# isl-org/Open3D

Measured on AMD Instinct MI355X. Metric: RGB-D frames/s, TSDF integrate with known poses (configs[1]: touch + activate + integrate into an 8 mm / 16^3 VoxelBlockGrid); the ICP + integrate + ray-cast loop (configs[2]) is in loop_frames_per_s (its first tracked frame untimed as warm-up; the whole run in loop_frames_per_s_with_first_frame), higher is better.
Workload: dtype f32; 1 GPU; block_count=50000, frames_per_launch=12, active_blocks=5745

## Files before the change

### open3d_amd/csrc/host/voxel_block_grid.cpp

```cpp

#include <cctype>
#include <chrono>
#include <cstdio>
#include <cstdlib>
#include <cstring>
#include <string>
#include <vector>

#include "../common.h"
#include "../npz.h"
#include "../stream_path.h"
#include "../sliced_path.h"
#include "../touch_device.h"
#include "../collectives.h"
#include "o3d_mi355x_host.h"

using namespace o3dmi;

struct o3dmi_vbg {
    float voxel_size = 0;
    int64_t block_resolution = 0;
    std::vector<std::string> attr_names;
    std::vector<int> attr_dtypes;
    std::vector<int> attr_channels;
// ... 1000 lines not shown
    int64_t seq = 0;
    int stamp = 0;
    const StreamFrame* frames = nullptr;
};

static StreamGroup MakeGroup(o3dmi_vbg* g, const StreamCommon& c,
                             const StreamFrame* frames, int n,
                             FrameFrontArgs* fa) {
    StreamGroup grp;
    grp.n = n;
    grp.seq = g->stream_seq;
    g->frame_stamp += 1;
    grp.stamp = g->frame_stamp;
    grp.frames = frames;
    const int par = (int)(grp.seq & 1);
    for (int f = 0; f < n; ++f) {
        FrameFrontArgs& a = fa[f];
        a.depth = (const uint16_t*)frames[f].depth;
        a.color = c.with_color ? (const uint8_t*)frames[f].color : nullptr;
        a.rows = c.depth_rows;
        a.cols = c.depth_cols;
        a.color_rows = c.color_rows;
        a.color_cols = c.color_cols;
        a.depth_intrinsic = c.depth_intrinsic;
        a.color_intrinsic = c.color_intrinsic ? c.color_intrinsic
                                              : c.depth_intrinsic;
        a.extrinsic = frames[f].extrinsic;
        a.resolution = (int)g->block_resolution;
        a.voxel_size = g->voxel_size;
        a.sdf_trunc = g->voxel_size * c.trunc;
        a.depth_scale = c.depth_scale;
        a.depth_max = c.depth_max;
        a.stride = 4;
        a.group_stamp = (unsigned long long)grp.stamp;
        a.group_bit = f;
        a.touch_plane = par;
        a.col_lut = g->prep_valid ? g->prep_col : nullptr;
        a.row_lut = g->prep_valid ? g->prep_row : nullptr;
        a.depth_div_short = g->prep_valid && g->prep_div_short;
        a.prep_identity = g->prep_valid && g->prep_identity;
        a.recs = g->recs[par][f];
        a.list = g->lists[par];
        a.list_capacity = g->lists_capacity;
        a.count = g->ring_counters + (grp.seq & 3);
        a.ready = g->ready[par];
        a.tickets = g->front_tickets + 16 * par;
        a.touch_status = (int*)g->stream_status + 4;
        a.prepare_only = false;
    }
    g->stream_seq += 1;
    g->size_bound = o3dmi_hash_capacity(g->block_hashmap);
    return grp;
}

static void MakeIntegArgs(o3dmi_vbg* g, const StreamCommon& c,
                          const StreamGroup& grp, bool prof,
                          IntegrateStreamArgs* ia) {
    const int par = (int)(grp.seq & 1);
    ia->n_frames = grp.n;
    ia->group_stamp = (unsigned long long)grp.stamp;
    ia->touch_plane = par;
    for (int f = 0; f < grp.n; ++f) {
        ia->recs[f] = g->recs[par][f];
        ia->extrinsic[f] = grp.frames[f].extrinsic;
    }
    ia->rows = c.depth_rows;
    ia->cols = c.depth_cols;
    ia->with_color = c.with_color;
    ia->list = g->lists[par];
    ia->ready = g->ready[par];
    ia->count = g->ring_counters + (grp.seq & 3);
    ia->list_capacity = g->lists_capacity;
    ia->grid_hint = g->last_count;
    ia->tsdf = (float*)o3dmi_hash_value_buffer(g->block_hashmap, c.ti);
    ia->weight = o3dmi_hash_value_buffer(g->block_hashmap, c.wi);
    ia->color = c.with_color ? o3dmi_hash_value_buffer(g->block_hashmap, c.ci)
                             : nullptr;
    ia->grid_dtype = c.grid_dtype;
    ia->depth_intrinsic = c.depth_intrinsic;
    ia->resolution = (int)g->block_resolution;
    ia->voxel_size = g->voxel_size;
    ia->sdf_trunc = g->voxel_size * c.trunc;
    ia->depth_max = c.depth_max;
    ia->zero_counter = g->ring_counters + ((grp.seq + 2) & 3);
    ia->size_host = (int*)g->stream_status;
    ia->status_stamp = grp.stamp;
    ia->prof_count = prof ? g->prof_counts + g->prof_max + g->prof_frames
                          : nullptr;
    ia->prof_frame_blocks = prof ? g->prof_counts + g->prof_frames : nullptr;
    ia->prof_map_size =
            prof ? g->prof_counts + 2 * g->prof_max + g->prof_frames : nullptr;
}

static bool StreamPathApplies(const o3dmi_vbg* g, int input_dtype) {
    int ti = g->AttrIndex("tsdf"), wi = g->AttrIndex("weight");
    return input_dtype == O3DMI_U16 && (g->block_resolution % 4) == 0 &&
           ti >= 0 && wi >= 0 && g->attr_dtypes[(size_t)ti] == O3DMI_F32;
}

static int WaitTouchReported(o3dmi_vbg* g, int stamp, hipStream_t s,
                             int* overflow) {
    const auto t0 = std::chrono::steady_clock::now();
    for (;;) {
        int st = PollStreamStatus(g, overflow);
        if (st) return st;
        if (*overflow != 0 || g->touch_seen_stamp - stamp >= 0) return O3DMI_OK;
        if (std::chrono::steady_clock::now() - t0 >
            std::chrono::milliseconds(20)) {
            O3DMI_HIP_CHECK(hipStreamSynchronize(s));
            if ((st = PollStreamStatus(g, overflow))) return st;
            return O3DMI_OK;
        }
    }
}

static int StreamIntegrate(o3dmi_vbg* g, const StreamCommon& c0,
                           const StreamFrame* frames, int n, int group,
                           hipStream_t s) {
    StreamCommon c = c0;
    if (group < 1) group = 1;
    if (group > kMaxGroup) group = kMaxGroup;
    c.frame_new = FrustumBlockBound(
            c.depth_intrinsic, c.depth_rows, c.depth_cols, c.depth_max,
            g->voxel_size * (float)g->block_resolution, 4);
    O3DMI_REQUIRE(c.frame_new > 0, "depth image too small");
    const int64_t group_new = c.frame_new * group;
    c.ti = g->AttrIndex("tsdf");
    c.wi = g->AttrIndex("weight");
    c.ci = g->AttrIndex("color");
    c.with_color = c.ci >= 0 && (int64_t)c.color_rows * c.color_cols > 0 &&
                   n > 0 && frames[0].color != nullptr;
    int st = GridDtype(g, &c.grid_dtype);
    if (st) return st;
    if ((st = EnsureStreamBuffers(g, c.depth_rows, c.depth_cols,
                                  c.frame_new * kMaxGroup)))
        return st;

    if ((st = EnsurePrepTables(g, c.depth_intrinsic, c.color_intrinsic,
                                      c.depth_rows, c.depth_cols,
                                      c.color_rows, c.color_cols,
                                      c.depth_scale, s))) {
        return st;
    }
    (void)PrefetchFastDivision(g->voxel_size * c.trunc, n == 1);
    static const bool strict_only =
            std::getenv("O3DMI_STRICT_CAPACITY") != nullptr;
    const bool allow_est = !strict_only && n > 1;

    struct Pending {
        int stamp, f0;
    };
    std::vector<Pending> pending;
    bool issued = false;
    StreamGroup cur;
    FrameFrontArgs fa[kMaxGroup];
    int f = 0;
    for (;;) {
        int overflow = 0;
        while (f < n && overflow == 0) {
            if (!issued) {
                Issue how;
                if ((st = StreamEnsureCapacity(g, group_new, allow_est, s,
                                               &how, &overflow)))
                    return st;
                if (overflow != 0) break;
                const int m = n - f < group ? n - f : group;
// ... 1876 lines not shown
```

### open3d_amd/csrc/stream_path.h

```cpp
#pragma once

#include "common.h"

namespace o3dmi {

constexpr int kMaxGroup = 16;
static_assert(kMaxGroup == kTouchBits, "one touch bit per frame of a group");
constexpr int kDefaultGroup = 8;
constexpr int kGroupChunk = 4;

struct alignas(16) FrameBlock {
    int slot, x, y, z;
};

struct alignas(16) ReadyEntry {
    unsigned long long key;
    int block_idx;
    unsigned bits;
};

struct alignas(8) PixelRec {
    float d;
    unsigned rgba;
};

struct FrameFrontArgs {
    const uint16_t* depth;
    const uint8_t* color;
    int rows, cols, color_rows, color_cols;
    const double* depth_intrinsic;
    const double* color_intrinsic;
    const double* extrinsic;
    int resolution;
    float voxel_size, sdf_trunc, depth_scale, depth_max;
    int stride;
    unsigned long long group_stamp;
    int group_bit;
    int touch_plane;
    const int* col_lut;
    const int* row_lut;
    bool depth_div_short;
    bool prep_identity;
    PixelRec* recs;
    FrameBlock* list;
    int64_t list_capacity;
    int* count;
    ReadyEntry* ready;
    int* tickets;
    int* touch_status;
    bool prepare_only;
};

struct IntegrateStreamArgs {
    int n_frames;
    unsigned long long group_stamp;
    int touch_plane;
    const PixelRec* recs[kMaxGroup];
    const double* extrinsic[kMaxGroup];
    int rows, cols;
    bool with_color;
    const FrameBlock* list;
    const ReadyEntry* ready;
    const int* count;
    int64_t list_capacity;
    int grid_hint;
    float* tsdf;
    void* weight;
    void* color;
    int grid_dtype;
    const double* depth_intrinsic;
    int resolution;
    float voxel_size, sdf_trunc, depth_max;
    int* zero_counter;
    int* size_host;
    int status_stamp;
    int* prof_count;
    int* prof_frame_blocks;
    int* prof_map_size;
};

int LaunchFrameStep(o3dmi_hash* block_hash, const FrameFrontArgs* fronts,
                    int n_fronts, const IntegrateStreamArgs* integ,
                    hipStream_t s);

int PrefetchFastDivision(float sdf_trunc, bool wait);

int RecoverOverflow(o3dmi_hash* block_hash, hipStream_t s, int64_t* wanted);

bool PrepTables(const double* depth_intrinsic, const double* color_intrinsic,
                int rows, int cols, int color_rows, int color_cols,
                float depth_scale, int* col, int* row);

int64_t FrustumBlockBound(const double* intrinsic, int rows, int cols,
                          float depth_max, float block_size, int stride);

}
```

### open3d_amd/csrc/vbg_stream.hip

```cpp

#include <cmath>

#include "common.h"
#include <cmath>
#include <cstdio>
#include <cstdlib>
#include <cstring>
#include <map>
#include <mutex>
#include <string>

#include "stream_path.h"
#include "sliced_path.h"
#include "touch_device.h"

#ifndef O3DMI_ABLATE_GATHER
#define O3DMI_ABLATE_GATHER 0
#endif

namespace o3dmi {
namespace {

template <typename T, int N, int A>
struct alignas(A) Vec {
    T v[N];
};

__device__ __forceinline__ float DivByConst(float a, float b, float y) {
    const float q0 = a * y;
    const float r = __builtin_fmaf(-b, q0, a);
    return __builtin_fmaf(r, y, q0);
}
struct PrepParams {
    Camera color_cam;
    int color_rows, color_cols;
    bool with_color;
};

constexpr int kTileKeys = 2048;

struct FrontShared {
    TouchParams p;
    PrepParams pp;
    const int* col_lut;
    const int* row_lut;
    bool depth_div_short;
    bool prep_identity;
    float inv_depth_scale;
    FrameBlock* list;
    int64_t list_capacity;
    int* out_count;
    ReadyEntry* ready;
    int* tickets;
    int* touch_status;
    int n_touch_total;
    unsigned long long group_stamp;
    int touch_plane;
    int n_touch_wg, n_prep_wg;
};
inline bool SameIntrinsics(const Camera& a, const Camera& b) {
    return a.fx == b.fx && a.fy == b.fy && a.cx == b.cx && a.cy == b.cy &&
           a.scale == b.scale;
}
inline bool SameGroup(const FrontShared& a, const FrontShared& b) {
    return SameIntrinsics(a.p.cam, b.p.cam) && a.p.rows == b.p.rows &&
           a.p.cols == b.p.cols && a.p.stride == b.p.stride &&
           a.p.rows_strided == b.p.rows_strided &&
           a.p.cols_strided == b.p.cols_strided &&
           a.p.block_size == b.p.block_size &&
           a.p.sdf_trunc == b.p.sdf_trunc &&
           a.p.depth_scale == b.p.depth_scale &&
           a.p.depth_max == b.p.depth_max &&
           SameIntrinsics(a.pp.color_cam, b.pp.color_cam) &&
           a.pp.color_rows == b.pp.color_rows &&
           a.pp.color_cols == b.pp.color_cols &&
           a.pp.with_color == b.pp.with_color && a.col_lut == b.col_lut &&
           a.row_lut == b.row_lut && a.depth_div_short == b.depth_div_short &&
           a.prep_identity == b.prep_identity &&
           a.inv_depth_scale == b.inv_depth_scale && a.list == b.list &&
           a.list_capacity == b.list_capacity && a.out_count == b.out_count &&
           a.ready == b.ready && a.tickets == b.tickets &&
           a.touch_status == b.touch_status &&
           a.n_touch_total == b.n_touch_total &&
           a.group_stamp == b.group_stamp && a.touch_plane == b.touch_plane &&
           a.n_touch_wg == b.n_touch_wg && a.n_prep_wg == b.n_prep_wg;
}
struct FrontFrame {
    float pose[3][4];
    const uint16_t* depth;
    const uint8_t* color;
    PixelRec* recs;
    int group_bit;
};

struct FrontParams {
    TouchParams p;
    PrepParams pp;
    const uint16_t* depth;
    const uint8_t* color;
    const int* col_lut;
    const int* row_lut;
    bool depth_div_short;
    bool prep_identity;
    float inv_depth_scale;
    PixelRec* recs;
    FrameBlock* list;
    int64_t list_capacity;
    int* out_count;
    ReadyEntry* ready;
    int* tickets;
    int* touch_status;
    int n_touch_total;
    unsigned long long group_stamp;
    int group_bit;
    int touch_plane;
// ... 104 lines not shown
                    __hip_atomic_store(fp.out_count, 0, __ATOMIC_RELAXED,
                                       __HIP_MEMORY_SCOPE_AGENT);
            }
            if (threadIdx.x == 0 && fp.touch_status) {
                const int top = __hip_atomic_load(&hv.counters[0],
                                                  __ATOMIC_RELAXED,
                                                  __HIP_MEMORY_SCOPE_AGENT);
                fp.touch_status[0] = top < hv.capacity ? top : hv.capacity;
                fp.touch_status[1] = overflow;
                fp.touch_status[2] = n;
                __hip_atomic_store(&fp.touch_status[3], (int)fp.group_stamp,
                                   __ATOMIC_RELEASE, __HIP_MEMORY_SCOPE_SYSTEM);
            }
            const auto make_entry = [&](int i) -> ReadyEntry {
                const unsigned long long* e =
                        reinterpret_cast<const unsigned long long*>(&list[i]);
                const unsigned long long lo = __hip_atomic_load(
                        e, __ATOMIC_RELAXED, __HIP_MEMORY_SCOPE_AGENT);
                const unsigned long long hi = __hip_atomic_load(
                        e + 1, __ATOMIC_RELAXED, __HIP_MEMORY_SCOPE_AGENT);
                const unsigned slot = (unsigned)lo;
                const int x = (int)(unsigned)(lo >> 32);
                const int y = (int)(unsigned)hi, z = (int)(unsigned)(hi >> 32);
                const int idx = __hip_atomic_load(&hv.slot_vals[slot],
                                                  __ATOMIC_RELAXED,
                                                  __HIP_MEMORY_SCOPE_AGENT);
                const unsigned long long word = __hip_atomic_load(
                        TouchWord(hv, slot, fp.touch_plane), __ATOMIC_RELAXED,
                        __HIP_MEMORY_SCOPE_AGENT);
                const bool own = (word >> kTouchBits) == fp.group_stamp;
                if (!own) atomicOr(&hv.counters[1], kErrTouchStamp);
                ReadyEntry re;
                re.key = PackKey(x, y, z);
                re.block_idx = idx;
                re.bits = own ? (unsigned)(word & ((1ull << kTouchBits) - 1ull))
                              : 0u;
                return re;
            };
            constexpr int kPerLane = 4;
            const int kSortable = kPerLane * (int)blockDim.x;
            __shared__ int s_bins[kTouchBits + 2];
            if (n <= kSortable) {
                if (threadIdx.x < kTouchBits + 2) s_bins[threadIdx.x] = 0;
                __syncthreads();
                ReadyEntry mine[kPerLane];
                int pc[kPerLane];
#pragma unroll
                for (int k = 0; k < kPerLane; ++k) {
                    const int i = (int)threadIdx.x + k * (int)blockDim.x;
                    pc[k] = -1;
                    if (i < n) {
                        mine[k] = make_entry(i);
                        pc[k] = __popc(mine[k].bits);
                    }
                }
#pragma unroll
                for (int k = 0; k < kPerLane; ++k)
                    if (pc[k] >= 0) atomicAdd(&s_bins[pc[k]], 1);
                __syncthreads();
                if (threadIdx.x == 0) {
                    int run = 0;
                    for (int b = kTouchBits; b >= 0; --b) {
                        const int c = s_bins[b];
                        s_bins[b] = run;
                        run += c;
                    }
                }
                __syncthreads();
#pragma unroll
                for (int k = 0; k < kPerLane; ++k)
                    if (pc[k] >= 0)
                        fp.ready[atomicAdd(&s_bins[pc[k]], 1)] = mine[k];
            } else {
                for (int i = threadIdx.x; i < n; i += blockDim.x)
                    fp.ready[i] = make_entry(i);
            }
        }
        return;
    }
    const int n_px = p.rows * p.cols;
    const int n_wg = fp.n_prep_wg;
    if (wg == n_touch_wg && threadIdx.x == 0) {
        PixelRec r;
        r.d = 0.0f;
        r.rgba = 0u;
        recs[n_px] = r;
    }
    if (fp.col_lut && fp.prep_identity) {
        const int n_groups = n_px >> 2;
        const int gstep = n_wg * blockDim.x;
        constexpr int kG = 4;
        for (int g0 = (wg - n_touch_wg) * blockDim.x + threadIdx.x;
             g0 < n_groups; g0 += kG * gstep) {
            uint2 dq[kG];
            unsigned cw[kG][3];
#pragma unroll
            for (int k = 0; k < kG; ++k) {
                const int g = g0 + k * gstep;
                const int gc = g < n_groups ? g : n_groups - 1;
                dq[k] = *reinterpret_cast<const uint2*>(depth + 4 * (int64_t)gc);
                if (pp.with_color) {
                    const unsigned* c = reinterpret_cast<const unsigned*>(
                            color + 12 * (int64_t)gc);
                    cw[k][0] = c[0];
                    cw[k][1] = c[1];
                    cw[k][2] = c[2];
                }
            }
#pragma unroll
            for (int k = 0; k < kG; ++k) {
                const int g = g0 + k * gstep;
                if (g >= n_groups) continue;
                const unsigned dv[4] = {dq[k].x & 0xffffu, dq[k].x >> 16,
                                        dq[k].y & 0xffffu, dq[k].y >> 16};
                unsigned rgba[4] = {0u, 0u, 0u, 0u};
                if (pp.with_color) {
                    rgba[0] = (cw[k][0] & 0xffffffu) | (1u << 24);
                    rgba[1] = ((cw[k][0] >> 24) | ((cw[k][1] & 0xffffu) << 8)) |
                              (1u << 24);
                    rgba[2] = ((cw[k][1] >> 16) | ((cw[k][2] & 0xffu) << 16)) |
                              (1u << 24);
                    rgba[3] = (cw[k][2] >> 8) | (1u << 24);
                }
                uint4 o[2];
                unsigned w[8];
#pragma unroll
                for (int j = 0; j < 4; ++j) {
                    const float df = (float)dv[j];
                    const float d =
                            fp.depth_div_short
                                    ? DivByConst(df, p.depth_scale,
                                                 fp.inv_depth_scale)
                                    : df / p.depth_scale;
                    w[2 * j] = __float_as_uint(d);
                    w[2 * j + 1] = rgba[j];
                }
                o[0] = make_uint4(w[0], w[1], w[2], w[3]);
                o[1] = make_uint4(w[4], w[5], w[6], w[7]);
                uint4* dst = reinterpret_cast<uint4*>(recs + 4 * (int64_t)g);
                dst[0] = o[0];
                dst[1] = o[1];
            }
        }
        return;
    }
    if (fp.col_lut) {
        const int* __restrict__ col_lut = fp.col_lut;
        const int* __restrict__ row_lut = fp.row_lut;
        const int step = n_wg * blockDim.x;
        const int step_v = step / p.cols, step_u = step - step_v * p.cols;
        for (int first = (wg - n_touch_wg) * blockDim.x + threadIdx.x;
             first < n_px; first += 4 * step) {
            int idx[4], uc[4], vc[4];
            float df[4];
#pragma unroll
            for (int k = 0; k < 4; ++k) {
                const int i = first + k * step;
                idx[k] = i < n_px ? i : n_px - 1;
                df[k] = (float)depth[idx[k]];
            }
            if (pp.with_color) {
                int vi = first / p.cols;
                int ui = first - vi * p.cols;
#pragma unroll
                for (int k = 0; k < 4; ++k) {
                    uc[k] = col_lut[ui];
                    vc[k] = row_lut[vi < p.rows ? vi : p.rows - 1];
                    ui += step_u;
                    vi += step_v;
                    if (ui >= p.cols) {
                        ui -= p.cols;
                        ++vi;
                    }
                }
            }
            unsigned rgba[4] = {0u, 0u, 0u, 0u};
            if (pp.with_color) {
                unsigned c0[4], c1[4], c2[4];
#pragma unroll
                for (int k = 0; k < 4; ++k) {
                    const bool has = (uc[k] | vc[k]) >= 0;
                    const uint8_t* in =
                            color + (has ? ((int64_t)vc[k] * pp.color_cols +
                                            uc[k]) * 3
                                         : 0);
                    c0[k] = in[0];
                    c1[k] = in[1];
                    c2[k] = in[2];
                }
#pragma unroll
                for (int k = 0; k < 4; ++k)
                    rgba[k] = (uc[k] | vc[k]) >= 0
                                      ? (c0[k] | (c1[k] << 8) | (c2[k] << 16) |
                                         (1u << 24))
                                      : 0u;
            }
#pragma unroll
            for (int k = 0; k < 4; ++k) {
                PixelRec r;
                r.d = fp.depth_div_short
                              ? DivByConst(df[k], p.depth_scale,
                                           fp.inv_depth_scale)
                              : df[k] / p.depth_scale;
                r.rgba = rgba[k];
                if (first + k * step < n_px) recs[idx[k]] = r;
            }
        }
        return;
    }
    for (int i = (wg - n_touch_wg) * blockDim.x + threadIdx.x; i < n_px;
         i += n_wg * blockDim.x) {
        const int vi = i / p.cols;
        const int ui = i - vi * p.cols;
        PixelRec r;
        r.d = (float)depth[i] / p.depth_scale;
        r.rgba = 0u;
        if (pp.with_color) {
            float x, y, z, uf, vf;
            p.cam.Unproject((float)ui, (float)vi, 1.0f, x, y, z);
            pp.color_cam.Project(x, y, z, uf, vf);
            if (InBoundary2D(uf, vf, pp.color_rows, pp.color_cols)) {
                int uc = (int)roundf(uf);
                int vc = (int)roundf(vf);
                const uint8_t* in =
                        color + ((int64_t)vc * pp.color_cols + uc) * 3;
                r.rgba = (unsigned)in[0] | ((unsigned)in[1] << 8) |
                         ((unsigned)in[2] << 16) | (1u << 24);
            }
        }
        recs[i] = r;
    }
}

struct IntegParams {
    Camera cam0;
    float ext[kMaxGroup][3][4];
    const PixelRec* recs[kMaxGroup];
    int n_frames;
    unsigned long long group_stamp;
    int touch_plane;
    int rows, cols, resolution;
    int res_shift;
    int cube;
    float sdf_trunc, depth_max;
    float inv_sdf_trunc;
    const FrameBlock* list;
    const ReadyEntry* ready;
    const int* count;
    int64_t list_capacity;
    float* tsdf;
    void* weight;
    void* color;
    int* zero_counter;
    int* size_host;
    int status_stamp;
    int* prof_count;
    unsigned long long* prof_items;
    int* prof_frame_blocks;
    int* prof_map_size;
    const uint16_t* raw_depth[kMaxGroup];
    const uint8_t* raw_color[kMaxGroup];
    float depth_scale, inv_depth_scale;
    bool depth_div_short;
    const ChunkEntry* entries;
    const IntegFrame* frame_tab;
};

__device__ __forceinline__ float RcpSmallInt(float b) {
    const float r0 = __builtin_amdgcn_rcpf(b);
    const float e = __builtin_fmaf(-b, r0, 1.0f);
    return __builtin_fmaf(e, r0, r0);
}

constexpr float kDivTiny = 1.0e-30f;

__device__ __forceinline__ float DivByConstGuarded(float a, float b, float y) {
    if (__builtin_amdgcn_ballot_w64(fabsf(a) < kDivTiny) != 0ull) return a / b;
    return DivByConst(a, b, y);
}

__global__ void VerifyDivKernel(float b, float y, unsigned max_bits,
                                int* __restrict__ mismatch) {
    int bad = 0;
    for (unsigned long long i = blockIdx.x * (unsigned long long)blockDim.x +
                                threadIdx.x;
         i <= max_bits; i += (unsigned long long)gridDim.x * blockDim.x) {
        const float a = __uint_as_float((unsigned)i);
        const float want_p = a / b, want_n = (-a) / b;
        const float got_p = DivByConstGuarded(a, b, y);
        const float got_n = DivByConstGuarded(-a, b, y);
        if (__float_as_uint(want_p) != __float_as_uint(got_p) ||
            __float_as_uint(want_n) != __float_as_uint(got_n))
            bad |= 1;
    }
    if (bad) atomicOr(mismatch, bad);
}
template <int kSteps>
__device__ __forceinline__ float RcpGuarded(float z) {
    const bool out = (__float_as_uint(z) - 0x21800000u) >= (0x5E000000u - 0x21800000u);
    if (__builtin_amdgcn_ballot_w64(out) != 0ull) return 1.0f / z;
    float r = __builtin_amdgcn_rcpf(z);
#pragma unroll
    for (int k = 0; k < kSteps; ++k) {
        const float e = __builtin_fmaf(-z, r, 1.0f);
        r = __builtin_fmaf(e, r, r);
    }
    return r;
}
__device__ __forceinline__ bool RcpOutOfRange(float z) {
    return (__float_as_uint(z) - 0x21800000u) >= (0x5E000000u - 0x21800000u);
}
template <int kSteps>
__device__ __forceinline__ float RcpNewton(float z) {
    float r = __builtin_amdgcn_rcpf(z);
#pragma unroll
    for (int k = 0; k < kSteps; ++k) {
        const float e = __builtin_fmaf(-z, r, 1.0f);
        r = __builtin_fmaf(e, r, r);
    }
    return r;
}
template <int kSteps>
__global__ void VerifyRcpZKernel(int* __restrict__ mismatch, int bit) {
    const unsigned lo = 0x21000000u, hi = 0x5E800000u;
    bool bad = false;
    for (unsigned long long i = lo + blockIdx.x * (unsigned long long)blockDim.x +
                                threadIdx.x;
         i <= hi; i += (unsigned long long)gridDim.x * blockDim.x) {
        const float z = __uint_as_float((unsigned)i);
        bad |= __float_as_uint(1.0f / z) !=
               __float_as_uint(RcpGuarded<kSteps>(z));
    }
    if (bad) atomicOr(mismatch, bit);
}

__global__ void VerifyRcpKernel(int* __restrict__ mismatch) {
    const int i = blockIdx.x * blockDim.x + threadIdx.x + 1;
    if (i > 65536) return;
    const float b = (float)i;
    if (__float_as_uint(1.0f / b) != __float_as_uint(RcpSmallInt(b)))
        atomicOr(mismatch, 2);
}

typedef float f2 __attribute__((ext_vector_type(2)));

__device__ __forceinline__ f2 Splat(float a) { return f2{a, a}; }
__device__ __forceinline__ f2 PkFma(f2 a, f2 b, f2 c) {
    return __builtin_elementwise_fma(a, b, c);
}

template <typename weight_t, typename color_t, bool kColor, int kDiv,
          int kChunk, int kP, bool kRaw = false, bool kLong = false>
__device__ __forceinline__ void IntegrateRoleWide(const HashView& hv,
                                                  const IntegParams& ip,
                                                  int wg, int n_wg,
                                                  int first_wg) {
    constexpr int kV = 2 * kP;
    constexpr int kVShift = kP == 2 ? 2 : 1;
    using FrameTabC = const IntegFrame __attribute__((address_space(4)));
    using ByteG = const char __attribute__((address_space(1)));
    using U16G = const uint16_t __attribute__((address_space(1)));
    typedef unsigned U2v __attribute__((ext_vector_type(2)));
    using U2G = const U2v __attribute__((address_space(1)));
    FrameTabC* const ftab = (FrameTabC*)ip.frame_tab;
    using TVec = Vec<float, kV, 4 * kV>;
    using WVec = Vec<weight_t, kV, kV * sizeof(weight_t)>;
    using CVec = Vec<color_t, 3 * kV, kV * sizeof(color_t)>;
    constexpr bool kU16 = sizeof(weight_t) == 2;
    float* __restrict__ tsdf_base = ip.tsdf;
    weight_t* __restrict__ weight_base = (weight_t*)ip.weight;
    color_t* __restrict__ color_base = (color_t*)ip.color;
    const FrameBlock* __restrict__ list = ip.list;
    int64_t n_blocks = *ip.count;
    if (n_blocks > ip.list_capacity) n_blocks = ip.list_capacity;

    if (wg == 0 && threadIdx.x == 0) {
        if (ip.zero_counter) *ip.zero_counter = 0;
        if (ip.prof_count) *ip.prof_count = (int)n_blocks;
        if (ip.prof_map_size) *ip.prof_map_size = hv.counters[0];
        if (ip.size_host) {
            ip.size_host[0] = hv.counters[0];
            ip.size_host[1] = hv.counters[1];
            ip.size_host[2] = (int)n_blocks;
            __hip_atomic_store(&ip.size_host[3], ip.status_stamp,
                               __ATOMIC_RELEASE, __HIP_MEMORY_SCOPE_SYSTEM);
        }
    }

    const int res = ip.resolution;
    const int res3 = res * res * res;
    const int quads_per_row = res >> kVShift;
    const int n_quads = res3 >> kVShift;
    const int parts = (n_quads + 255) >> 8;
    const int res_shift = ip.res_shift;
    int frame_blocks = 0;

    const int xcd = (first_wg + wg) & 7;
    const int first_of_xcd = (xcd - first_wg) & 7;
    const int rank = (wg - first_of_xcd) >> 3;
    const int n_on_xcd =
            first_of_xcd < n_wg ? ((n_wg - 1 - first_of_xcd) >> 3) + 1 : 0;
    const int64_t first_b = xcd;
    const int64_t blocks_on_xcd = (n_blocks + 7 - xcd) >> 3;
    const int64_t n_items = blocks_on_xcd * parts;
    const unsigned sentinel_off =
            (unsigned)(ip.rows * ip.cols) * (unsigned)sizeof(PixelRec);
    const unsigned row_bytes = (unsigned)ip.cols * (unsigned)sizeof(PixelRec);
    const float vscale = ip.cam0.scale;
    const float fx = ip.cam0.fx, fyk = ip.cam0.fy;
    const float cx = ip.cam0.cx, cy = ip.cam0.cy;
    const unsigned u_max_bits = __float_as_uint(ip.cols - 1.0f);
    const unsigned v_max_bits = __float_as_uint(ip.rows - 1.0f);
    const unsigned last_col8 = (unsigned)(ip.rows * ip.cols) * 3u - 8u;

    for (int64_t m = rank; m < n_items; m += n_on_xcd) {
        int64_t kb;
        int part;
        if (res_shift >= 0) {
            const int ps0 = 3 * res_shift - kVShift - 8;
            const int ps = ps0 > 0 ? ps0 : 0;
            kb = m >> ps;
            part = (int)(m & ((1 << ps) - 1));
        } else {
            kb = m / parts;
            part = (int)(m - kb * parts);
        }
        const int64_t b = first_b + (kb << 3);
        unsigned long long item_t0 = 0ull;
        if constexpr (kLong)
            if (ip.prof_items && threadIdx.x == 0) item_t0 = wall_clock64();
        int xb, yb, zb, block_idx;
        unsigned bits;
        unsigned long_bits = 0u;
        if constexpr (kLong) {
            const ChunkEntry* __restrict__ ce = ip.entries + b;
            const unsigned klo =
                    __builtin_amdgcn_readfirstlane((unsigned)ce->key);
            const unsigned khi =
                    __builtin_amdgcn_readfirstlane((unsigned)(ce->key >> 32));
            const unsigned long long key =
                    ((unsigned long long)khi << 32) | klo;
            xb = (int)((key >> 42) & 0x1FFFFFull) - kKeyBias;
            yb = (int)((key >> 21) & 0x1FFFFFull) - kKeyBias;
            zb = (int)(key & 0x1FFFFFull) - kKeyBias;
            block_idx = __builtin_amdgcn_readfirstlane(ce->block_idx);
            long_bits = ce->bits[threadIdx.x & (kChunkWords - 1)];
            unsigned any = 0u;
#pragma unroll
            for (int w = 0; w < kChunkWords; ++w) {
                const unsigned bw =
                        (unsigned)__builtin_amdgcn_readlane((int)long_bits, w);
// ... 26 lines not shown
            block_idx = __builtin_amdgcn_readfirstlane(re.block_idx);
            bits = __builtin_amdgcn_readfirstlane(re.bits);
        } else {
            const FrameBlock fb = list[b];
            const int slot = __builtin_amdgcn_readfirstlane(fb.slot);
            xb = __builtin_amdgcn_readfirstlane(fb.x);
            yb = __builtin_amdgcn_readfirstlane(fb.y);
            zb = __builtin_amdgcn_readfirstlane(fb.z);
            block_idx = __builtin_amdgcn_readfirstlane(hv.slot_vals[slot]);
            const unsigned long long word =
                    *TouchWord(hv, slot, ip.touch_plane);
            const bool own = (word >> kTouchBits) == ip.group_stamp;
            if (!own && threadIdx.x == 0 && part == 0)
                atomicOr(&hv.counters[1], kErrTouchStamp);
            bits = __builtin_amdgcn_readfirstlane(
                    own ? (unsigned)(word & ((1ull << kTouchBits) - 1ull))
                        : 0u);
        }
        const int64_t block_base = (int64_t)block_idx * res3;
        if (!kLong && part == 0 && threadIdx.x == 0 && ip.prof_frame_blocks)
            frame_blocks += __popc(bits);
        if constexpr (!kLong) {
            const int n_set = __popc(bits);
            if (n_set >= 3 * ip.n_frames / 4) __builtin_amdgcn_s_setprio(3);
            else if (n_set >= ip.n_frames / 2) __builtin_amdgcn_s_setprio(2);
            else if (n_set >= ip.n_frames / 4) __builtin_amdgcn_s_setprio(1);
            else __builtin_amdgcn_s_setprio(0);
        }
        int opaque = 0;
        asm volatile("" : "+s"(opaque));

        const int q = (part << 8) + threadIdx.x;
        if (q >= n_quads || bits == 0u) continue;
        int qx, yv, zv;
        int lin_q = q;
        if (res_shift - kVShift >= 2 && ip.cube) {
            const int nx = res_shift - kVShift;
            const unsigned uq = (unsigned)q;
            unsigned rest = uq >> 6;
            const unsigned qx_hi = rest & ((1u << (nx - 2)) - 1u);
            rest >>= (nx - 2);
            const unsigned y_hi = rest & ((1u << (res_shift - 2)) - 1u);
            rest >>= (res_shift - 2);
            qx = (int)((uq & 3u) | (qx_hi << 2));
            yv = (int)(((uq >> 2) & 3u) | (y_hi << 2));
            zv = (int)(((uq >> 4) & 3u) | (rest << 2));
            lin_q = (((zv << res_shift) | yv) << nx) | qx;
        } else if (res_shift >= 0) {
            qx = q & (quads_per_row - 1);
            const int row = q >> (res_shift - kVShift);
            yv = row & (res - 1);
            zv = row >> res_shift;
        } else {
            qx = q % quads_per_row;
            const int row = q / quads_per_row;
            yv = row % res;
            zv = row / res;
        }
        const int x0 = xb * res + (qx << kVShift);
        const float fy = (float)(yb * res + yv);
        const float fz = (float)(zb * res + zv);
        const int64_t lin0 = block_base + ((int64_t)lin_q << kVShift);

        const TVec t4 = *reinterpret_cast<const TVec*>(tsdf_base + lin0);
        float ts[kV];
        float wf[kV];
        float cf[kV][3];
#pragma unroll
        for (int v = 0; v < kV; ++v) ts[v] = t4.v[v];
        {
            const WVec w4 = *reinterpret_cast<const WVec*>(weight_base + lin0);
#pragma unroll
            for (int v = 0; v < kV; ++v) wf[v] = (float)w4.v[v];
            if constexpr (kColor) {
                const CVec c12 =
                        *reinterpret_cast<const CVec*>(color_base + 3 * lin0);
#pragma unroll
                for (int v = 0; v < kV; ++v)
#pragma unroll
                    for (int i = 0; i < 3; ++i)
                        cf[v][i] = (float)c12.v[3 * v + i];
            }
        }

        const float ys = fy * vscale, zs = fz * vscale;
        f2 xs[kP];
#pragma unroll
        for (int p = 0; p < kP; ++p)
            xs[p] = f2{(float)(x0 + 2 * p), (float)(x0 + 2 * p + 1)} * vscale;
        bool touched = false;
        struct Round {
            f2 zc[kChunk][kP];
            PixelRec rec[kChunk][kV];
            unsigned chi[kRaw && kColor ? kChunk : 1][kV];
            unsigned csh[kRaw && kColor ? kChunk : 1][kV];
            uint16_t dr[kRaw ? kChunk : 1][kV];
            unsigned in_mask;
            unsigned cbits;
        };
        auto round_bits = [&](int c0) -> unsigned {
            if constexpr (kLong)
                return ((unsigned)__builtin_amdgcn_readlane((int)long_bits,
                                                            c0 >> 5) >>
                        (c0 & 31)) &
                       ((1u << kChunk) - 1u);
            else
                return (bits >> c0) & ((1u << kChunk) - 1u);
        };
        auto issue = [&](int c0, Round& R) {
        R.in_mask = 0u;
#pragma unroll
        for (int fk = 0; fk < kChunk; ++fk) {
            const int f = c0 + fk;
            if (!((R.cbits >> fk) & 1u)) continue;
            float e_tab[3][4];
            if constexpr (kLong) {
#pragma unroll
                for (int i = 0; i < 3; ++i)
#pragma unroll
                    for (int j = 0; j < 4; ++j) e_tab[i][j] = ftab[f].ext[i][j];
            }
            const float(&e)[3][4] =
                    kLong ? e_tab
                          : *reinterpret_cast<const float(*)[3][4]>(
                                    &ip.ext[kLong ? 0 : f][0][0] + opaque);
            const char* __restrict__ recs = reinterpret_cast<const char*>(
                    kRaw ? nullptr
                         : (kLong ? (const void*)ftab[f].recs
                                  : *(&ip.recs[kLong ? 0 : f] + opaque)));
            ByteG* __restrict__ dimg = (ByteG*)(
                    kLong ? (const void*)ftab[f].depth
                          : (kRaw ? *(&ip.raw_depth[kLong ? 0 : f] + opaque)
                                  : nullptr));
            ByteG* __restrict__ cimg = (ByteG*)(
                    kLong ? (const void*)ftab[f].color
                          : (kRaw ? *(&ip.raw_color[kLong ? 0 : f] + opaque)
                                  : nullptr));
            const float y0 = ys * e[0][1], z0 = zs * e[0][2];
            const float y1 = ys * e[1][1], z1 = zs * e[1][2];
            const float y2 = ys * e[2][1], z2 = zs * e[2][2];
            f2 xc[kP], yc[kP];
#pragma unroll
            for (int p = 0; p < kP; ++p) {
                xc[p] = xs[p] * e[0][0] + y0 + z0 + e[0][3];
                yc[p] = xs[p] * e[1][0] + y1 + z1 + e[1][3];
                R.zc[fk][p] = xs[p] * e[2][0] + y2 + z2 + e[2][3];
            }
            f2 inv_z[kP];
            const bool out = RcpOutOfRange(R.zc[fk][0].x) ||
                             RcpOutOfRange(R.zc[fk][kP - 1].y);
            if (kDiv < 2 || __builtin_amdgcn_ballot_w64(out) != 0ull) {
#pragma unroll
                for (int p = 0; p < kP; ++p)
                    inv_z[p] = f2{1.0f / R.zc[fk][p].x, 1.0f / R.zc[fk][p].y};
            } else {
#pragma unroll
                for (int p = 0; p < kP; ++p) {
                    f2 r = f2{__builtin_amdgcn_rcpf(R.zc[fk][p].x),
                              __builtin_amdgcn_rcpf(R.zc[fk][p].y)};
                    r = PkFma(PkFma(-R.zc[fk][p], r, Splat(1.0f)), r, r);
                    inv_z[p] = r;
                }
            }
#pragma unroll
            for (int p = 0; p < kP; ++p) {
                const f2 u = xc[p] * fx * inv_z[p] + cx;
                const f2 v = yc[p] * fyk * inv_z[p] + cy;
#pragma unroll
                for (int h = 0; h < 2; ++h) {
                    const float uh = h ? u.y : u.x, vh = h ? v.y : v.x;
                    const bool in = __float_as_uint(vh) <= v_max_bits &&
                                    __float_as_uint(uh) <= u_max_bits;
                    if constexpr (kRaw) {
                        const unsigned pix =
                                in ? __umul24((unsigned)(int)vh,
                                              (unsigned)ip.cols) +
                                             (unsigned)(int)uh
                                   : 0u;
                        R.in_mask |= (in ? 1u : 0u) << (fk * kV + 2 * p + h);
                        PixelRec r;
                        R.dr[fk][2 * p + h] = *(U16G*)(dimg + 2u * pix);
                        r.rgba = 0u;
                        if constexpr (kColor) {
                            const unsigned b3 = 3u * pix;
                            unsigned al = b3 & ~3u;
                            al = al < last_col8 ? al : last_col8;
                            const U2v q = *(U2G*)(cimg + al);
                            r.rgba = q.x;
                            R.chi[fk][2 * p + h] = q.y;
                            R.csh[fk][2 * p + h] = (b3 - al) * 8u;
                        }
                        R.rec[fk][2 * p + h] = r;
                    } else {
                    unsigned off =
                            __umul24((unsigned)(int)vh, row_bytes) +
                            (unsigned)(int)uh * (unsigned)sizeof(PixelRec);
#if O3DMI_ABLATE_GATHER
                    off = __builtin_amdgcn_readfirstlane(in ? off
                                                            : sentinel_off);
                    R.rec[fk][2 * p + h] =
                            *reinterpret_cast<const PixelRec*>(recs + off);
#else
                    R.rec[fk][2 * p + h] = *reinterpret_cast<const PixelRec*>(
                            recs + (in ? off : sentinel_off));
#endif
                    }
                }
            }
        }

        };
        auto convert_depth = [&](int fk, Round& R) {
#pragma unroll
            for (int p = 0; p < kP; ++p) {
                f2 a = f2{(float)R.dr[kRaw ? fk : 0][2 * p],
                          (float)R.dr[kRaw ? fk : 0][2 * p + 1]};
                f2 q;
                if (ip.depth_div_short) {
                    const f2 q0 = a * ip.inv_depth_scale;
                    const f2 r = PkFma(Splat(-ip.depth_scale), q0, a);
                    q = PkFma(r, Splat(ip.inv_depth_scale), q0);
                } else {
                    q = f2{a.x / ip.depth_scale, a.y / ip.depth_scale};
                }
                R.rec[fk][2 * p].d =
                        ((R.in_mask >> (fk * kV + 2 * p)) & 1u) ? q.x : 0.0f;
                R.rec[fk][2 * p + 1].d =
                        ((R.in_mask >> (fk * kV + 2 * p + 1)) & 1u) ? q.y : 0.0f;
            }
        };
        auto apply = [&](int c0, Round& R) {
#pragma unroll
        for (int fk = 0; fk < kChunk; ++fk) {
            if (!((R.cbits >> fk) & 1u)) continue;
            if constexpr (kRaw) convert_depth(fk, R);
#pragma unroll
            for (int p = 0; p < kP; ++p) {
#pragma unroll
                for (int h = 0; h < 2; ++h) {
                    const float dh = R.rec[fk][2 * p + h].d;
                    const float zh = h ? R.zc[fk][p].y : R.zc[fk][p].x;
                    const float sh = dh - zh;
                    const bool ok = !(dh <= 0) && !(dh > ip.depth_max) &&
                                    !(zh <= 0) && !(sh < -ip.sdf_trunc);
                    if (!ok) continue;
                    touched = true;
                    float cl;
                    asm("v_min_f32 %0, %1, %2"
                        : "=v"(cl)
                        : "s"(ip.sdf_trunc), "v"(sh));
                    float sd;
                    if (kDiv < 1 || fabsf(cl) < kDivTiny)
                        sd = cl / ip.sdf_trunc;
                    else
                        sd = DivByConst(cl, ip.sdf_trunc, ip.inv_sdf_trunc);
                    const int vx = 2 * p + h;
                    const float weight = wf[vx];
                    const float wsum = weight + 1.0f;
                    float inv_wsum;
                    if constexpr (kU16 && kDiv >= 1) inv_wsum = RcpSmallInt(wsum);
                    else inv_wsum = 1.0f / wsum;
                    const float t_new = (weight * ts[vx] + sd) * inv_wsum;
                    ts[vx] = t_new;
                    if constexpr (kColor) {
                        unsigned rg = R.rec[fk][2 * p + h].rgba;
                        if constexpr (kRaw)
                            rg = (unsigned)((((unsigned long long)
                                                      R.chi[fk][2 * p + h]
                                              << 32) | rg) >>
                                            R.csh[fk][2 * p + h]);
                        if (kRaw || (rg >> 24)) {
#pragma unroll
                            for (int i = 0; i < 3; ++i) {
                                const float in =
                                        (float)((rg >> (8 * i)) & 0xffu);
                                float c_new =
                                        (weight * cf[vx][i] + in) * inv_wsum;
                                if constexpr (sizeof(color_t) == 2)
                                    c_new = truncf(c_new);
                                cf[vx][i] = c_new;
                            }
                        }
                    }
                    wf[vx] = wsum;
                    if constexpr (kU16) {
                        if (wsum >= 65536.0f) wf[vx] = 0.0f;
                    }
                }
            }
        }
        };
        auto round_drained = [] { __builtin_amdgcn_s_waitcnt(0x0F70); };
        if constexpr (kLong) {
#pragma nounroll
            for (int c0 = 0; c0 < ip.n_frames; c0 += kChunk) {
                Round r;
                r.cbits = round_bits(c0);
                if (r.cbits == 0u) continue;
                issue(c0, r);
                apply(c0, r);
                round_drained();
            }
        } else {
#pragma nounroll
            for (int c0 = 0; c0 < kMaxGroup; c0 += kChunk) {
                Round r;
                r.cbits = round_bits(c0);
                if (r.cbits == 0u) continue;
                issue(c0, r);
                apply(c0, r);
                round_drained();
            }
        }
        if (touched) {
            TVec t_out;
            WVec w4;
#pragma unroll
            for (int p = 0; p < kP; ++p) {
                t_out.v[2 * p] = ts[2 * p];
                t_out.v[2 * p + 1] = ts[2 * p + 1];
                w4.v[2 * p] = (weight_t)wf[2 * p];
                w4.v[2 * p + 1] = (weight_t)wf[2 * p + 1];
            }
            *reinterpret_cast<TVec*>(tsdf_base + lin0) = t_out;
            *reinterpret_cast<WVec*>(weight_base + lin0) = w4;
            if constexpr (kColor) {
                CVec c12;
#pragma unroll
                for (int p = 0; p < kP; ++p)
#pragma unroll
                    for (int i = 0; i < 3; ++i) {
                        c12.v[6 * p + i] = (color_t)cf[2 * p][i];
                        c12.v[6 * p + 3 + i] = (color_t)cf[2 * p + 1][i];
                    }
                *reinterpret_cast<CVec*>(color_base + 3 * lin0) = c12;
            }
        }
        if constexpr (kLong) {
            if (ip.prof_items && threadIdx.x == 0) {
                int n_set = 0;
#pragma unroll
                for (int w = 0; w < kChunkWords; ++w)
                    n_set += __popc((unsigned)__builtin_amdgcn_readlane(
                            (int)long_bits, w));
                unsigned long long* o = ip.prof_items + (b * parts + part) * 4;
                o[0] = item_t0;
                o[1] = wall_clock64();
                o[2] = ((unsigned long long)n_set << 32) |
                       (unsigned)__builtin_amdgcn_s_getreg((31 << 11) | 4);
                o[3] = ((unsigned long long)(unsigned)xcd << 32) | (unsigned)wg;
            }
        }
    }
    if (frame_blocks) atomicAdd(ip.prof_frame_blocks, frame_blocks);
}

struct StepParams {
    HashView hv;
    FrontShared fshared;
    FrontFrame front[kMaxGroup];
    IntegParams integ;
    int n_fronts;
    int front_wg;
};
static_assert(sizeof(StepParams) <= 4096, "kernel arguments are limited to 4 KB");


#ifndef O3DMI_RAW_CHUNK
#define O3DMI_RAW_CHUNK 4
#endif
#ifndef O3DMI_RAW_WAVES
#define O3DMI_RAW_WAVES 5
#endif
// ... 177 lines not shown
}

static void CanonicalPrincipalPoint(Camera& c) {
    if (c.cx == 0.0f) c.cx = 0.0f;
    if (c.cy == 0.0f) c.cy = 0.0f;
}

int LaunchFrameStep(o3dmi_hash* bh, const FrameFrontArgs* fronts, int n_fronts,
                    const IntegrateStreamArgs* a, hipStream_t s) {
    O3DMI_REQUIRE((n_fronts > 0 && fronts) || a, "nothing to launch");
    O3DMI_REQUIRE(n_fronts >= 0 && n_fronts <= kMaxGroup, "bad group size");
    StepParams sp = {};
    sp.hv = bh->view;
    sp.n_fronts = n_fronts;
    int n_int_wg = 0;
    int grid_dtype = O3DMI_U16;
    bool col = false;
    int fast_div = 0;
    static const double eye4[16] = {1, 0, 0, 0, 0, 1, 0, 0,
                                    0, 0, 1, 0, 0, 0, 0, 1};
    for (int i = 0; i < n_fronts; ++i) {
        const FrameFrontArgs* f = &fronts[i];
        O3DMI_REQUIRE(f->group_bit >= 0 && f->group_bit < kMaxGroup &&
                              (f->group_stamp > 0 || f->prepare_only),
                      "bad group bit / stamp");
        const TouchParams tp = MakeTouchParams(
                f->depth_intrinsic, f->extrinsic, f->rows, f->cols, f->stride,
                f->resolution, f->voxel_size, f->sdf_trunc, f->depth_scale,
                f->depth_max);
        FrontFrame& ff = sp.front[i];
        std::memcpy(ff.pose, tp.cam.e, sizeof(ff.pose));
        ff.depth = f->depth;
        ff.color = f->color;
        ff.recs = f->recs;
        ff.group_bit = f->group_bit;
        FrontShared fs = {};
        fs.p = tp;
        fs.pp.color_cam = Camera::Make(f->color_intrinsic ? f->color_intrinsic
                                                          : f->depth_intrinsic,
                                       eye4, 1.0f);
        fs.pp.color_rows = f->color_rows;
        fs.pp.color_cols = f->color_cols;
        fs.pp.with_color = f->color != nullptr;
        fs.col_lut = f->col_lut;
        fs.row_lut = f->col_lut ? f->row_lut : nullptr;
        fs.depth_div_short = f->depth_div_short;
        fs.prep_identity = f->col_lut && f->prep_identity &&
                           (f->cols % 4) == 0 && f->rows == f->color_rows &&
                           f->cols == f->color_cols;
        fs.inv_depth_scale = 1.0f / f->depth_scale;
        fs.list = f->list;
        fs.list_capacity = f->list_capacity;
        fs.out_count = f->count;
        fs.ready = f->ready;
        fs.tickets = f->ready ? f->tickets : nullptr;
        fs.touch_status = f->ready ? f->touch_status : nullptr;
        fs.group_stamp = f->group_stamp;
        fs.touch_plane = f->touch_plane & 1;
        fs.n_touch_wg = f->prepare_only
                                ? 0
                                : ((tp.cols_strided + 15) / 16) *
                                          ((tp.rows_strided + 15) / 16);
        fs.n_prep_wg = (f->rows * f->cols + kBlock * 16 - 1) / (kBlock * 16);
        if (fs.n_prep_wg < 1) fs.n_prep_wg = 1;
        fs.n_touch_total = fs.n_touch_wg * n_fronts;
        if (i == 0) {
            sp.fshared = fs;
            sp.front_wg = fs.n_touch_wg + fs.n_prep_wg;
        } else {
            O3DMI_REQUIRE(SameGroup(sp.fshared, fs),
                          "frames of one launch must share image size, "
                          "intrinsics, scales and their group");
        }
    }
    if (a) {
        O3DMI_REQUIRE(a->resolution % 4 == 0,
                      "frame-stream path needs block_resolution % 4 == 0");
        O3DMI_REQUIRE(a->n_frames >= 1 && a->n_frames <= kMaxGroup,
                      "bad group size");
        IntegParams& ip = sp.integ;
        ip.n_frames = a->n_frames;
        ip.group_stamp = a->group_stamp;
        ip.touch_plane = a->touch_plane & 1;
        for (int f = 0; f < a->n_frames; ++f) {
            const Camera cf = Camera::Make(a->depth_intrinsic, a->extrinsic[f],
                                           a->voxel_size);
            if (f == 0) {
                ip.cam0 = cf;
                CanonicalPrincipalPoint(ip.cam0);
            }
            std::memcpy(ip.ext[f], cf.e, sizeof(ip.ext[f]));
            ip.recs[f] = a->recs[f];
            ip.raw_depth[f] = nullptr;
            ip.raw_color[f] = nullptr;
        }
        ip.rows = a->rows;
        ip.cols = a->cols;
        ip.resolution = a->resolution;
        ip.res_shift = -1;
        for (int sh = 2; sh < 12; ++sh)
            if ((1 << sh) == a->resolution) ip.res_shift = sh;
        ip.cube = LaneCube(ip.res_shift);
        ip.sdf_trunc = a->sdf_trunc;
        ip.depth_max = a->depth_max;
        fast_div = VerifyFastDivision(a->sdf_trunc, &ip.inv_sdf_trunc);
        ip.list = a->list;
        ip.ready = a->ready;
        ip.count = a->count;
        ip.list_capacity = a->list_capacity;
        ip.tsdf = a->tsdf;
        ip.weight = a->weight;
        ip.color = a->color;
        ip.zero_counter = a->zero_counter;
        ip.size_host = a->size_host;
        ip.status_stamp = a->status_stamp;
        ip.prof_count = a->prof_count;
        ip.prof_frame_blocks = a->prof_frame_blocks;
        ip.prof_map_size = a->prof_map_size;
        const int n_quads =
                (a->resolution * a->resolution * a->resolution) >> 1;
        const int parts = (n_quads + 255) >> 8;
        int64_t g = ((int64_t)a->grid_hint + (a->grid_hint >> 2) + 64) * parts;
        const int64_t g_max = (int64_t)kCUs * 32;
        if (g > g_max) g = g_max;
        if (g < kCUs) g = kCUs;
        n_int_wg = (int)g;
        grid_dtype = a->grid_dtype;
        col = a->with_color && a->color != nullptr;
    }
    dim3 grid((unsigned)(n_fronts * sp.front_wg + n_int_wg)), block(256);
#define O3DMI_LAUNCH_STEP(WT, VT, COLOR)                                      \
    do {                                                                      \
        if (fast_div == 2)                                                    \
            hipLaunchKernelGGL((FrameStepKernel<WT, VT, COLOR, 2>), grid,     \
                               block, 0, s, sp);                              \
        else                                                                  \
            hipLaunchKernelGGL((FrameStepKernel<WT, VT, COLOR, 0>), grid,     \
                               block, 0, s, sp);                              \
    } while (0)
    if (grid_dtype == O3DMI_U16) {
        if (col) O3DMI_LAUNCH_STEP(uint16_t, uint16_t, true);
        else O3DMI_LAUNCH_STEP(uint16_t, uint16_t, false);
    } else {
        if (col) O3DMI_LAUNCH_STEP(float, float, true);
        else O3DMI_LAUNCH_STEP(float, float, false);
    }
#undef O3DMI_LAUNCH_STEP
    O3DMI_HIP_CHECK(hipGetLastError());
    return O3DMI_OK;
}

int LaunchChunkIntegrate(o3dmi_hash* bh, const ChunkIntegrateArgs& a,
                         hipStream_t s) {
    O3DMI_REQUIRE(a.resolution % 4 == 0 && a.n_frames >= 1 &&
                          a.n_frames <= kChunkFrames && a.frames &&
                          a.entries && a.count && a.depth_scale > 0,
                  "chunk integrate: bad arguments");
    ChunkParams cp = {};
    cp.hv = bh->view;
    IntegParams& ip = cp.integ;
    ip.n_frames = a.n_frames;
    static const double eye4[16] = {1, 0, 0, 0, 0, 1, 0, 0,
                                    0, 0, 1, 0, 0, 0, 0, 1};
    ip.cam0 = Camera::Make(a.depth_intrinsic, eye4, a.voxel_size);
    CanonicalPrincipalPoint(ip.cam0);
    ip.rows = a.rows;
    ip.cols = a.cols;
    ip.resolution = a.resolution;
    ip.res_shift = -1;
    for (int sh = 2; sh < 12; ++sh)
        if ((1 << sh) == a.resolution) ip.res_shift = sh;
    ip.cube = LaneCube(ip.res_shift);
    ip.sdf_trunc = a.sdf_trunc;
    ip.depth_max = a.depth_max;
    const int fast_div =
            VerifyFastDivision(a.sdf_trunc, &ip.inv_sdf_trunc, true);
    if (fast_div != 2) {
        SetLastError("chunk integrate: the short division forms are not "
                     "proven for this truncation distance (O3DMI_EXACT_DIV?) "
                     "-- use the replicated block touch");
        return O3DMI_ERR_UNSUPPORTED;
    }
    ip.list = nullptr;
    ip.ready = nullptr;
    ip.entries = a.entries;
    ip.frame_tab = a.frames;
    ip.count = a.count;
    ip.list_capacity = a.entries_cap;
// ... 93 lines not shown
```

Baseline: 161,300 frames/s.

## Fold depth validity into prepared records and specialize short-weight integrate path

The prep stage now writes -inf for invalid or out-of-range depths, so the integrate kernel's fast-division variant can drop its per-sample depth>0 and depth_max tests and the tiny-value division guard. Host-side checks on depth_scale, sdf_trunc and pose magnitude decide whether this folded path is safe; if they fail, the fast-division variant is disabled. A wave-uniform test also picks a short-form update that skips the u16 weight-wrap reset and uses an FMA for the color blend when no lane can wrap or overflow. The aim is fewer ALU ops and branches per voxel-frame sample, at the cost of more template instantiations, code size and host-side validation logic.

```diff
diff --git a/open3d_amd/csrc/host/voxel_block_grid.cpp b/open3d_amd/csrc/host/voxel_block_grid.cpp
--- a/open3d_amd/csrc/host/voxel_block_grid.cpp
+++ b/open3d_amd/csrc/host/voxel_block_grid.cpp
@@ -1106,6 +1106,7 @@
     ia->voxel_size = g->voxel_size;
     ia->sdf_trunc = g->voxel_size * c.trunc;
     ia->depth_max = c.depth_max;
+    ia->depth_scale = c.depth_scale;
     ia->zero_counter = g->ring_counters + ((grp.seq + 2) & 3);
     ia->size_host = (int*)g->stream_status;
     ia->status_stamp = grp.stamp;
diff --git a/open3d_amd/csrc/integrate_checks.h b/open3d_amd/csrc/integrate_checks.h
--- /dev/null
+++ b/open3d_amd/csrc/integrate_checks.h
@@ -0,0 +1,37 @@
+#pragma once
+
+#include <cmath>
+
+namespace o3dmi {
+
+constexpr float kDivTiny = 1.0e-30f;
+
+constexpr double kFoldCoordPerRes = 1048577.0;
+constexpr double kFoldTransformBound = 0x1p100;
+
+inline bool DepthFoldPoseOk(const float e[3][4], float voxel_size,
+                            int resolution, float sdf_trunc) {
+    if (!std::isfinite(voxel_size) || !std::isfinite(sdf_trunc) ||
+        resolution <= 0)
+        return false;
+    const double c = kFoldCoordPerRes * (double)resolution *
+                     std::fabs((double)voxel_size);
+    for (int i = 0; i < 3; ++i) {
+        double s = 0.0;
+        for (int j = 0; j < 4; ++j) {
+            if (!std::isfinite(e[i][j])) return false;
+            s += std::fabs((double)e[i][j]) * (j < 3 ? c : 1.0);
+        }
+        if (!(s <= kFoldTransformBound)) return false;
+    }
+    return true;
+}
+
+inline bool SdfDivGuardRedundant(float depth_scale, float sdf_trunc) {
+    if (!(depth_scale > 0.0f) || !std::isfinite(depth_scale)) return false;
+    const float min_depth = 1.0f / depth_scale;
+    return min_depth >= 0x1p-75f && sdf_trunc >= kDivTiny &&
+           std::isfinite(sdf_trunc);
+}
+
+}
diff --git a/open3d_amd/csrc/stream_path.h b/open3d_amd/csrc/stream_path.h
--- a/open3d_amd/csrc/stream_path.h
+++ b/open3d_amd/csrc/stream_path.h
@@ -71,6 +71,7 @@
     const double* depth_intrinsic;
     int resolution;
     float voxel_size, sdf_trunc, depth_max;
+    float depth_scale;
     int* zero_counter;
     int* size_host;
     int status_stamp;
diff --git a/open3d_amd/csrc/vbg_stream.hip b/open3d_amd/csrc/vbg_stream.hip
--- a/open3d_amd/csrc/vbg_stream.hip
+++ b/open3d_amd/csrc/vbg_stream.hip
@@ -9,7 +9,9 @@
 #include <map>
 #include <mutex>
 #include <string>
-
+#include <type_traits>
+
+#include "integrate_checks.h"
 #include "stream_path.h"
 #include "sliced_path.h"
 #include "touch_device.h"
@@ -31,6 +33,10 @@
     const float r = __builtin_fmaf(-b, q0, a);
     return __builtin_fmaf(r, y, q0);
 }
+__device__ __forceinline__ float RecordDepth(float d, float depth_max) {
+    return (!(d <= 0) && !(d > depth_max)) ? d : -__builtin_inff();
+}
+
 struct PrepParams {
     Camera color_cam;
     int color_rows, color_cols;
@@ -301,7 +307,7 @@
     const int n_wg = fp.n_prep_wg;
     if (wg == n_touch_wg && threadIdx.x == 0) {
         PixelRec r;
-        r.d = 0.0f;
+        r.d = -__builtin_inff();
         r.rgba = 0u;
         recs[n_px] = r;
     }
@@ -351,7 +357,7 @@
                                     ? DivByConst(df, p.depth_scale,
                                                  fp.inv_depth_scale)
                                     : df / p.depth_scale;
-                    w[2 * j] = __float_as_uint(d);
+                    w[2 * j] = __float_as_uint(RecordDepth(d, p.depth_max));
                     w[2 * j + 1] = rgba[j];
                 }
                 o[0] = make_uint4(w[0], w[1], w[2], w[3]);
@@ -417,10 +423,11 @@
 #pragma unroll
             for (int k = 0; k < 4; ++k) {
                 PixelRec r;
-                r.d = fp.depth_div_short
-                              ? DivByConst(df[k], p.depth_scale,
-                                           fp.inv_depth_scale)
-                              : df[k] / p.depth_scale;
+                r.d = RecordDepth(fp.depth_div_short
+                                          ? DivByConst(df[k], p.depth_scale,
+                                                       fp.inv_depth_scale)
+                                          : df[k] / p.depth_scale,
+                                  p.depth_max);
                 r.rgba = rgba[k];
                 if (first + k * step < n_px) recs[idx[k]] = r;
             }
@@ -432,7 +439,7 @@
         const int vi = i / p.cols;
         const int ui = i - vi * p.cols;
         PixelRec r;
-        r.d = (float)depth[i] / p.depth_scale;
+        r.d = RecordDepth((float)depth[i] / p.depth_scale, p.depth_max);
         r.rgba = 0u;
         if (pp.with_color) {
             float x, y, z, uf, vf;
@@ -491,7 +498,6 @@
     return __builtin_fmaf(e, r0, r0);
 }
 
-constexpr float kDivTiny = 1.0e-30f;
 
 __device__ __forceinline__ float DivByConstGuarded(float a, float b, float y) {
     if (__builtin_amdgcn_ballot_w64(fabsf(a) < kDivTiny) != 0ull) return a / b;
@@ -586,6 +592,7 @@
     using WVec = Vec<weight_t, kV, kV * sizeof(weight_t)>;
     using CVec = Vec<color_t, 3 * kV, kV * sizeof(color_t)>;
     constexpr bool kU16 = sizeof(weight_t) == 2;
+    constexpr bool kFold = kDiv >= 2 && !kRaw && !kLong;
     float* __restrict__ tsdf_base = ip.tsdf;
     weight_t* __restrict__ weight_base = (weight_t*)ip.weight;
     color_t* __restrict__ color_base = (color_t*)ip.color;
@@ -778,6 +785,23 @@
                         cf[v][i] = (float)c12.v[3 * v + i];
             }
         }
+        bool c_small = !(kColor && sizeof(color_t) == 2), may_wrap = true;
+        if constexpr (kU16 && kFold) {
+            float w_max = wf[0];
+#pragma unroll
+            for (int v = 1; v < kV; ++v) w_max = fmaxf(w_max, wf[v]);
+            may_wrap = __builtin_amdgcn_ballot_w64(
+                               w_max + (float)ip.n_frames >= 65536.0f) != 0ull;
+            if constexpr (kColor && sizeof(color_t) == 2) {
+                float c_max = cf[0][0];
+#pragma unroll
+                for (int v = 0; v < kV; ++v)
+#pragma unroll
+                    for (int i = 0; i < 3; ++i) c_max = fmaxf(c_max, cf[v][i]);
+                c_small = __builtin_amdgcn_ballot_w64(c_max > 255.0f) == 0ull;
+            }
+        }
+        const bool short_item = kU16 && kFold && c_small && !may_wrap;
 
         const float ys = fy * vscale, zs = fz * vscale;
         f2 xs[kP];
@@ -925,11 +949,8 @@
                         ((R.in_mask >> (fk * kV + 2 * p + 1)) & 1u) ? q.y : 0.0f;
             }
         };
-        auto apply = [&](int c0, Round& R) {
-#pragma unroll
-        for (int fk = 0; fk < kChunk; ++fk) {
-            if (!((R.cbits >> fk) & 1u)) continue;
-            if constexpr (kRaw) convert_depth(fk, R);
+        auto update = [&](int fk, Round& R, auto short_form) {
+            constexpr bool kShort = decltype(short_form)::value;
 #pragma unroll
             for (int p = 0; p < kP; ++p) {
 #pragma unroll
@@ -937,8 +958,11 @@
                     const float dh = R.rec[fk][2 * p + h].d;
                     const float zh = h ? R.zc[fk][p].y : R.zc[fk][p].x;
                     const float sh = dh - zh;
-                    const bool ok = !(dh <= 0) && !(dh > ip.depth_max) &&
-                                    !(zh <= 0) && !(sh < -ip.sdf_trunc);
+                    const bool ok =
+                            kFold ? !(zh <= 0) && !(sh < -ip.sdf_trunc)
+                                  : !(dh <= 0) && !(dh > ip.depth_max) &&
+                                            !(zh <= 0) &&
+                                            !(sh < -ip.sdf_trunc);
                     if (!ok) continue;
                     touched = true;
                     float cl;
@@ -946,7 +970,7 @@
                         : "=v"(cl)
                         : "s"(ip.sdf_trunc), "v"(sh));
                     float sd;
-                    if (kDiv < 1 || fabsf(cl) < kDivTiny)
+                    if (kDiv < 1 || (!kFold && fabsf(cl) < kDivTiny))
                         sd = cl / ip.sdf_trunc;
                     else
                         sd = DivByConst(cl, ip.sdf_trunc, ip.inv_sdf_trunc);
@@ -970,8 +994,14 @@
                             for (int i = 0; i < 3; ++i) {
                                 const float in =
                                         (float)((rg >> (8 * i)) & 0xffu);
-                                float c_new =
-                                        (weight * cf[vx][i] + in) * inv_wsum;
+                                float c_new;
+                                if constexpr (kShort)
+                                    c_new = __builtin_fmaf(weight, cf[vx][i],
+                                                           in) *
+                                            inv_wsum;
+                                else
+                                    c_new = (weight * cf[vx][i] + in) *
+                                            inv_wsum;
                                 if constexpr (sizeof(color_t) == 2)
                                     c_new = truncf(c_new);
                                 cf[vx][i] = c_new;
@@ -979,12 +1009,25 @@
                         }
                     }
                     wf[vx] = wsum;
-                    if constexpr (kU16) {
+                    if constexpr (kU16 && !kShort) {
                         if (wsum >= 65536.0f) wf[vx] = 0.0f;
                     }
                 }
             }
-        }
+        };
+        auto apply = [&](int c0, Round& R) {
+        auto frames = [&](auto short_form) {
+#pragma unroll
+            for (int fk = 0; fk < kChunk; ++fk) {
+                if (!((R.cbits >> fk) & 1u)) continue;
+                if constexpr (kRaw) convert_depth(fk, R);
+                update(fk, R, short_form);
+            }
+        };
+        if (short_item)
+            frames(std::true_type());
+        else
+            frames(std::false_type());
         };
         auto round_drained = [] { __builtin_amdgcn_s_waitcnt(0x0F70); };
         if constexpr (kLong) {
@@ -1328,9 +1371,12 @@
         ip.n_frames = a->n_frames;
         ip.group_stamp = a->group_stamp;
         ip.touch_plane = a->touch_plane & 1;
+        bool fold = SdfDivGuardRedundant(a->depth_scale, a->sdf_trunc);
         for (int f = 0; f < a->n_frames; ++f) {
             const Camera cf = Camera::Make(a->depth_intrinsic, a->extrinsic[f],
                                            a->voxel_size);
+            fold = fold && DepthFoldPoseOk(cf.e, a->voxel_size, a->resolution,
+                                           a->sdf_trunc);
             if (f == 0) {
                 ip.cam0 = cf;
                 CanonicalPrincipalPoint(ip.cam0);
@@ -1350,6 +1396,7 @@
         ip.sdf_trunc = a->sdf_trunc;
         ip.depth_max = a->depth_max;
         fast_div = VerifyFastDivision(a->sdf_trunc, &ip.inv_sdf_trunc);
+        if (!fold) fast_div = 0;
         ip.list = a->list;
         ip.ready = a->ready;
         ip.count = a->count;
```

New measurement: 171,900 frames/s (median of 6 runs). 6.5% higher.
